# maropu/hivemall

Measured on AMD Instinct MI355X. Metric: rows/sec (node) FFM on Criteo-shaped sparse at 1/2/4/8 MI355X; logloss parity, higher is better.
Workload: dtype fp32

## Files before the change

### csrc/kernels/ffm.hip

```cpp
#include <type_traits>

#include "common.h"

namespace {

struct FFMParams {
    int B, F;
    int num_features, num_fields, Kp;
    int classification;
    int train;
    int use_linear, use_bias, norm;
    int reload;
    int gstride;
    int vpad;
    int tail16;
    int gfstride;
    int sstride;
    int fstride;
    long long vfe;
    uint32_t seed;
    float eta0, eps, lambda_v;
    float alpha, beta, lambda1, lambda2;
    float min_target, max_target;
    const void* reserved;
    int32_t* defer;
    int list_mode;
    int lin_defer;
    long long lstride;
    int lpack;
    int lin_atomic;
    const int32_t* hidx;
    const int32_t* hot_id;
    float* hacc;
    int nhot;
    int hacc_on;
    float* bias_sh;
    int bias_s;
    int bias_every;
};

#define LW(p, i) ((p)[(size_t)(i) * (size_t)P.lstride])

__device__ __forceinline__ float ftrl_weight(float z, float n, float alpha, float beta,
                                             float l1, float l2) {
    if (fabsf(z) <= l1) return 0.f;
    const float s = z > 0.f ? 1.f : -1.f;
    return -(z - s * l1) / ((beta + sqrtf(n)) / alpha + l2);
}

__device__ __forceinline__ float ftrl_update(float* __restrict__ z, float* __restrict__ n,
                                             float w, float g, float alpha, float beta,
                                             float l1, float l2) {
    const float n0 = *n;
    const float n1 = n0 + g * g;
    const float sigma = (sqrtf(n1) - sqrtf(n0)) / alpha;
    const float z1 = *z + g - sigma * w;
    *z = z1;
    *n = n1;
    return ftrl_weight(z1, n1, alpha, beta, l1, l2);
}

__device__ __forceinline__ float bias_w0(const FFMParams& P, const float* bias) {
    const float z = __hip_atomic_load(bias + 1, __ATOMIC_RELAXED, __HIP_MEMORY_SCOPE_AGENT);
    const float n = __hip_atomic_load(bias + 2, __ATOMIC_RELAXED, __HIP_MEMORY_SCOPE_AGENT);
    return ftrl_weight(z, n, P.alpha, P.beta, 0.f, 0.f);
}

__device__ __forceinline__ void bias_update(const FFMParams& P, float g, float* bias) {
    const float z0 = __hip_atomic_load(bias + 1, __ATOMIC_RELAXED, __HIP_MEMORY_SCOPE_AGENT);
    const float n0 = __hip_atomic_load(bias + 2, __ATOMIC_RELAXED, __HIP_MEMORY_SCOPE_AGENT);
    const float w = ftrl_weight(z0, n0, P.alpha, P.beta, 0.f, 0.f);
    const float sigma = (sqrtf(n0 + g * g) - sqrtf(n0)) / P.alpha;
    const float dz = g - sigma * w;
    atomicAdd(bias + 1, dz);
    atomicAdd(bias + 2, g * g);
    bias[0] = ftrl_weight(z0 + dz, n0 + g * g, P.alpha, P.beta, 0.f, 0.f);
}

__device__ __forceinline__ void bias_update_sh(const FFMParams& P, float g, float z0, float n0, float* sh,
                                               float* acc) {
    const float w = ftrl_weight(z0, n0, P.alpha, P.beta, 0.f, 0.f);
    const float sigma = (sqrtf(n0 + g * g) - sqrtf(n0)) / P.alpha;
    const float dz = g - sigma * w;
    atomicAdd(sh, dz);
    atomicAdd(sh + 1, g * g);
    acc[0] += dz;
    acc[1] += g * g;
}

constexpr int HD_SIZE = 2048;
constexpr int HD12_SIZE = 1024;
constexpr int HACC_STRIDE = 32;
constexpr int HACC_GRID = 2048;
constexpr int HACC_GRID12 = 2304;

__device__ __forceinline__ uint32_t hash3(uint32_t a, uint32_t b, uint32_t c) {
    uint32_t h = a * 0x9E3779B1u ^ (b + 0x7F4A7C15u) * 0x85EBCA77u ^ c * 0xC2B2AE3Du;
    h ^= h >> 15; h *= 0x2C1B3C6Du; h ^= h >> 12; h *= 0x297A2D39u; h ^= h >> 15;
    return h;
}

template <bool BF>
__device__ __forceinline__ float4 ld_chunk(const void* base, size_t off) {
    if constexpr (BF) {
        const uint2 q = *reinterpret_cast<const uint2*>(reinterpret_cast<const uint16_t*>(base) + off);
        return make_float4(__uint_as_float(q.x << 16), __uint_as_float(q.x & 0xFFFF0000u),
                           __uint_as_float(q.y << 16), __uint_as_float(q.y & 0xFFFF0000u));
    } else {
        return *reinterpret_cast<const float4*>(reinterpret_cast<const float*>(base) + off);
    }
}

template <bool BF>
__device__ __forceinline__ typename std::conditional<BF, uint2, float4>::type ld_raw(const void* base, size_t off) {
    if constexpr (BF) return *reinterpret_cast<const uint2*>(reinterpret_cast<const uint16_t*>(base) + off);
    else return *reinterpret_cast<const float4*>(reinterpret_cast<const float*>(base) + off);
}

template <bool BF, typename T>
__device__ __forceinline__ float4 to_f4(const T& q) {
    if constexpr (BF) {
        return make_float4(__uint_as_float(q.x << 16), __uint_as_float(q.x & 0xFFFF0000u),
                           __uint_as_float(q.y << 16), __uint_as_float(q.y & 0xFFFF0000u));
    } else {
        return q;
    }
}

template <bool BF>
__device__ __forceinline__ void st_chunk(void* base, size_t off, float4 v, uint32_t rnd) {
    if constexpr (BF) {
        const uint32_t r2 = rnd * 0x9E3779B1u + 0x632BE5ABu;
        const uint32_t lo = hm::pack_bf16x2_sr(v.x, rnd, v.y, rnd >> 16);
        const uint32_t hi = hm::pack_bf16x2_sr(v.z, r2, v.w, r2 >> 16);
        *reinterpret_cast<uint2*>(reinterpret_cast<uint16_t*>(base) + off) = make_uint2(lo, hi);
    } else {
        *reinterpret_cast<float4*>(reinterpret_cast<float*>(base) + off) = v;
    }
}

struct SlotMeta {
    int i, f;
    float x;
};

// ... 662 lines not shown
    if constexpr (PIN) asm("" : "+v"(m0), "+v"(m1), "+v"(m2), "+v"(m3));
    return m0 + m1 + m2 + m3;
}

constexpr int SG32_TRAIN = 1;

template <int NS, typename OT, int TPB = 256, int ATOM = 0, int KV = 1, int KEEP = 0, int LT = 0, int CFG = 0>
__global__ __launch_bounds__(TPB) __attribute__((amdgpu_waves_per_eu(TPB / 128))) void ffm_pipe_sg32_kernel(
    FFMParams P, const int32_t* __restrict__ idx, const int32_t* __restrict__ fld,
    const float* __restrict__ val, const float* __restrict__ y, void* __restrict__ Vt,
    float* __restrict__ Gt, float* __restrict__ w, float* __restrict__ wz, float* __restrict__ wn,
    float* __restrict__ bias, float* __restrict__ pred_out, float* __restrict__ loss_out)
{
    constexpr bool SPEC = (CFG & SG32_TRAIN) != 0;
    static_assert(!SPEC || (ATOM == 0 && KV == 1 && KEEP >= 2 && sizeof(OT) == 4 && TPB == 256),
                  "SG32_TRAIN: the default fp32 k <= 4 training launch only");
#define c_train (SPEC || P.train)
#define c_linear (SPEC || P.use_linear)
#define c_lpack (SPEC || P.lpack)
#define c_ldefer (SPEC || P.lin_defer)
#define c_bias (!SPEC && P.use_bias)
#define c_fld (SPEC || fld)
#define c_val (SPEC || val)
#define c_hacc (SPEC ? LT != 0 : P.hacc_on)
    __shared__ __attribute__((aligned(16))) float4 s_rv[NS * TPB * KV];
    __shared__ __attribute__((aligned(16))) float s_rg[NS * TPB];
    __shared__ __attribute__((aligned(16))) float4 s_t[NS * TPB * KV];
    __shared__ __attribute__((aligned(16))) int4 s_m[2][48];
    __shared__ __attribute__((aligned(16))) int s_mr[2][3][48];
    __shared__ __attribute__((aligned(16))) float s_lin[2][3][48];
    __shared__ __attribute__((aligned(16))) float4 s_lin4[2][48];
    __shared__ float s_red[TPB / 64 + 2];
    __shared__ int s_rep[TPB / 64];
    __shared__ float s_bias[4];
    __shared__ float s_bcur[2];
    __shared__ float2 s_hd[LT ? HD_SIZE : 1];
    __shared__ __attribute__((aligned(16))) float4 s_hacc[LT ? 2 : 1][48];
    __shared__ __attribute__((aligned(16))) int s_nh[LT ? 2 : 1][48];
    const int F = P.F;
    const int FF = F * F;
    const int tid = threadIdx.x, lane = tid & 63;
    const int wave = SPEC ? __builtin_amdgcn_readfirstlane(tid >> 6) : tid >> 6;
    constexpr int W_META = 1, W_LIN = 2, W_DMA = 3;
    const OT vfs = (OT)P.fstride * (16u * KV);
    const OT gfs = (OT)P.gstride * 4u;
    const int G = (int)gridDim.x;
    const int bid = (int)blockIdx.x;
    char* vb = reinterpret_cast<char*>(Vt);
    char* gb = reinterpret_cast<char*>(Gt);
    if constexpr (LT != 0) {
        for (int t = tid; t < HD_SIZE; t += TPB) s_hd[t] = make_float2(0.f, 0.f);
    }
    int nh = -1, kh = -1;

    int ab[NS];
    uint32_t okm = 0u;
#pragma unroll
    for (int j = 0; j < NS; ++j) {
        const int s = tid + j * TPB;
        if constexpr (SPEC) {
            const int a = s < FF ? s / F : 0, b = s < FF ? s % F : 0;
            ab[j] = (a << 4) | (b << 10) | ((s < FF ? b * F + a : s) << 16);
            okm |= (uint32_t)(s >= FF) << j | (uint32_t)(s >= FF || a == b) << (8 + j) | (uint32_t)(a < b) << (16 + j);
        } else {
            ab[j] = s < FF ? (s / F) | ((s % F) << 8) : 0;
        }
    }
#define SA(j) (SPEC ? (ab[j] >> 4) & 0x3F : ab[j] & 0xFF)
#define SB(j) (SPEC ? (ab[j] >> 10) & 0x3F : ab[j] >> 8)
#define ST(j) (SPEC ? ab[j] >> 16 : (SB(j) * F + SA(j)) * KV)

    auto dma_meta = [&](int bf, int row) {
        if (wave == W_DMA && lane < F && row < P.B) {
            const size_t o = (size_t)row * F + lane;
            __builtin_amdgcn_global_load_lds((glb_ptr_t)(idx + o), (lds_ptr_t)&s_mr[bf][0][0], 4, 0, 0);
            if (c_fld) __builtin_amdgcn_global_load_lds((glb_ptr_t)(fld + o), (lds_ptr_t)&s_mr[bf][1][0], 4, 0, 0);
            if (c_val) __builtin_amdgcn_global_load_lds((glb_ptr_t)(val + o), (lds_ptr_t)&s_mr[bf][2][0], 4, 0, 0);
        }
    };
    auto publish_meta = [&](int bf) {
        if (wave == W_META) {
            float sq = 0.f;
            if (lane < F) {
                int ri = s_mr[bf][0][lane];
                int rf = c_fld ? s_mr[bf][1][lane] : lane;
                float rx = c_val ? __int_as_float(s_mr[bf][2][lane]) : 1.f;
                if (ri < 0 || ri >= P.num_features || rf < 0 || rf >= P.num_fields) { ri = -1; rx = 0.f; rf = 0; }
                const int hb = SPEC && ri >= 0 ? (int)((uint32_t)ri * (uint32_t)vfs) : 0;
                s_m[bf][lane] = make_int4(ri, rf, __float_as_int(rx), hb);
                sq = rx * rx;
            }
            const float tot = hm::wave_sum_uniform(sq);
            if (lane == 0) s_red[TPB / 64 + bf] = (P.norm && tot > 0.f) ? rsqrtf(tot) : 1.f;
        }
    };
    auto slot = [&](int bf, int j, OT& ov, OT& og, float& xab) -> uint32_t {
        const int4 ma = s_m[bf][SA(j)], mb = s_m[bf][SB(j)];
        const bool ok = (ma.x | mb.x) >= 0 && tid + j * TPB < FF;
        const bool live = ok && SA(j) != SB(j);
        const OT i = ok ? (OT)(uint32_t)ma.x : (OT)0, f = ok ? (OT)(uint32_t)mb.y : (OT)0;
        ov = i * vfs + f * (16u * KV);
        og = i * gfs + f * 4u;
        xab = live ? __int_as_float(ma.z) * __int_as_float(mb.z) : 0.f;
        return live ? 1u : (ok ? 2u : 0u);
    };
    OT kov[KEEP ? NS : 1], kog[KEEP ? NS : 1], nov[KEEP ? NS : 1], nog[KEEP ? NS : 1];
// ... 9 lines not shown
                const int4 ma = s_m[bf][SA(j)], mb = s_m[bf][SB(j)];
                const int both = ma.x | mb.x;
                const bool ok = (both | (int)(okm << (31 - j))) >= 0;
                const bool live = (both | (int)(okm << (23 - j))) >= 0;
                const OT ib = ok ? (OT)(uint32_t)ma.w : (OT)0, f = ok ? (OT)(uint32_t)mb.y : (OT)0;
                OT f4 = f * 4u;
                asm("" : "+v"(f4));
                nov[j] = ib + f * 16u;
                nog[j] = ib + f4;
                nxab[j] = live ? __int_as_float(ma.z) * __int_as_float(mb.z) : 0.f;
                nwr |= (uint32_t)ok << j;
                eq |= (uint32_t)(ma.x == mb.x || ma.y == mb.y) << j;
                __builtin_amdgcn_global_load_lds((glb_ptr_t)(vb + nov[j]), (lds_ptr_t)(s_rv + j * TPB + wave * 64), 16, 0, 0);
                __builtin_amdgcn_global_load_lds((glb_ptr_t)(gb + nog[j]), (lds_ptr_t)(s_rg + j * TPB + wave * 64), 4, 0, 0);
            }
            nlive = nwr & ~(okm >> 8);
            if (P.defer) nrep = (int)(eq & nwr & (okm >> 16));
            return;
        }
#pragma unroll
        for (int j = 0; j < NS; ++j) {
            OT ov, og;
            float xab;
            const uint32_t k = slot(bf, j, ov, og, xab);
            if constexpr (KEEP) {
                nov[j] = ov;
                nog[j] = og;
                nxab[j] = xab;
                nlive |= (k & 1u) << j;
                nwr |= (uint32_t)(k != 0u) << j;
                if (P.defer) nrep |= (int)slot_repeats(SA(j), SB(j), s_m[bf][SA(j)], s_m[bf][SB(j)]);
            }
#pragma unroll
            for (int q = 0; q < KV; ++q)
                __builtin_amdgcn_global_load_lds((glb_ptr_t)(vb + ov + 16u * q),
                                                 (lds_ptr_t)(s_rv + (q * NS + j) * TPB + wave * 64), 16, 0, 0);
            __builtin_amdgcn_global_load_lds((glb_ptr_t)(gb + og), (lds_ptr_t)(s_rg + j * TPB + wave * 64), 4, 0, 0);
        }
    };
    auto keep_rotate = [&]() {
        if constexpr (KEEP) {
#pragma unroll
            for (int j = 0; j < NS; ++j) { kov[j] = nov[j]; kog[j] = nog[j]; kxab[j] = nxab[j]; }
            klive = nlive; kwr = nwr; krep = nrep;
        }
    };
    const int nlin = (c_linear && c_ldefer) ? ((c_lpack || !c_train) ? 1 + (LT != 0) : 3) : 0;
    auto dma_lin = [&](int bf) {
        if (c_linear && wave == W_LIN && lane < F) {
            const int i = max(s_m[bf][lane].x, 0);
            if (c_lpack) {
                __builtin_amdgcn_global_load_lds((glb_ptr_t)&LW(w, i), (lds_ptr_t)&s_lin4[bf][0], 16, 0, 0);
                if constexpr (LT != 0)
                    __builtin_amdgcn_global_load_lds((glb_ptr_t)(P.hacc + HACC_STRIDE * max(nh, 0)), (lds_ptr_t)&s_hacc[bf][0], 16, 0, 0);
                return;
            }
            __builtin_amdgcn_global_load_lds((glb_ptr_t)&LW(w, i), (lds_ptr_t)&s_lin[bf][0][0], 4, 0, 0);
            if (c_train) {
                __builtin_amdgcn_global_load_lds((glb_ptr_t)&LW(wz, i), (lds_ptr_t)&s_lin[bf][1][0], 4, 0, 0);
                __builtin_amdgcn_global_load_lds((glb_ptr_t)&LW(wn, i), (lds_ptr_t)&s_lin[bf][2][0], 4, 0, 0);
            }
        }
    };

    int row = bid;
    if (row >= P.B) return;
    if (tid == 0) { s_bcur[0] = 0.f; s_bcur[1] = 0.f; }
    dma_meta(0, row);
    __builtin_amdgcn_s_waitcnt(0x0F70);
    bar_raw();
    publish_meta(0);
    bar_raw();
    dma_slots(0);
    keep_rotate();
    if constexpr (LT != 0) {
        if (wave == W_LIN && lane < F) nh = s_m[0][lane].x >= 0 ? P.hidx[s_m[0][lane].x] : -1;
    }
    dma_lin(0);
    kh = nh;
    dma_meta(1, row + G);

    float4 fv[NS][KV];
    float fg[NS];
    OT fo[NS];
    uint32_t fwd = 0u;
    const bool bsh = c_bias && P.bias_sh;
    int bit = 0;
    float bz = 0.f, bn = 0.f;
    if (bsh && wave == W_META && lane < P.bias_s) {
        bz = __hip_atomic_load(P.bias_sh + lane * 32, __ATOMIC_RELAXED, __HIP_MEMORY_SCOPE_AGENT);
        bn = __hip_atomic_load(P.bias_sh + lane * 32 + 1, __ATOMIC_RELAXED, __HIP_MEMORY_SCOPE_AGENT);
    }
    for (int cur = 0; row < P.B; row += G, cur ^= 1) {
        const int nxt = cur ^ 1;
        const bool more = row + G < P.B;
        if constexpr (SPEC) asm volatile("" : "+v"(okm));
        if (wave == W_LIN && nlin == 3) __builtin_amdgcn_s_waitcnt(0x0F73);
        else if (wave == W_LIN && nlin == 2) __builtin_amdgcn_s_waitcnt(0x0F72);
        else if (wave == W_LIN && nlin == 1) __builtin_amdgcn_s_waitcnt(0x0F71);
        else __builtin_amdgcn_s_waitcnt(0x0F70);
        bar_raw();
        const bool bre = bsh && bit > 0 && (bit % P.bias_every) == 0;
        float nbz = bz, nbn = bn;
        if (bre && wave == W_META && lane < P.bias_s) {
            nbz = __hip_atomic_load(P.bias_sh + lane * 32, __ATOMIC_RELAXED, __HIP_MEMORY_SCOPE_AGENT);
            nbn = __hip_atomic_load(P.bias_sh + lane * 32 + 1, __ATOMIC_RELAXED, __HIP_MEMORY_SCOPE_AGENT);
        }
// ... 168 lines not shown
                            atomicAdd(vp + 4 * q + 2, e1.x);
                            atomicAdd(vp + 4 * q + 3, e1.y);
                        }
                        atomicAdd(reinterpret_cast<float*>(gb + og), gs - cg[j]);
                    }
                    continue;
                }
#pragma unroll
                for (int q = 0; q < KV; ++q) *reinterpret_cast<float4*>(vb + ov + 16u * q) = fv[j][q];
                *reinterpret_cast<float*>(gb + og) = fg[j];
            }
            if (mi >= 0) {
                if (c_linear) {
                    const float lz = hot ? hz : (c_lpack ? s_lin4[cur][lane].y : s_lin[cur][1][lane]);
                    const float ln = hot ? hn : (c_lpack ? s_lin4[cur][lane].z : s_lin[cur][2][lane]);
                    const float g = kappa * mx * scale;
                    const float n1 = ln + g * g;
                    const float z1 = lz + g - (sqrtf(n1) - sqrtf(ln)) / P.alpha * lw;
                    const float w1 = ftrl_weight(z1, n1, P.alpha, P.beta, P.lambda1, P.lambda2);
                    if (LT && hot) {
                        const float2 d = s_hd[kh];
                        s_hd[kh] = make_float2(d.x + (g - (sqrtf(n1) - sqrtf(ln)) / P.alpha * lw), d.y + g * g);
                    } else if (ATOM == 1) {
                        atomicAdd(&LW(wz, mi), z1 - lz);
                        atomicAdd(&LW(wn, mi), g * g);
                        LW(w, mi) = w1;
                    } else if (c_lpack) {
                        *reinterpret_cast<float4*>(&LW(w, mi)) = make_float4(w1, z1, n1, s_lin4[cur][lane].w);
                    } else {
                        LW(wz, mi) = z1;
                        LW(wn, mi) = n1;
                        LW(w, mi) = w1;
                    }
                }
            }
            if (c_bias && tid == 0) {
                if (bsh) bias_update_sh(P, kappa, s_bias[1], s_bias[2], P.bias_sh + (blockIdx.x % P.bias_s) * 32, s_bcur);
                else bias_update(P, kappa, bias);
            }
        }
        if constexpr (LT != 0) {
            if (more && wave == W_LIN && lane < F) nh = s_nh[nxt][lane];
        }
        if (more) dma_lin(nxt);
        kh = nh;
        keep_rotate();
        bz = nbz;
        bn = nbn;
        ++bit;
    }
    __builtin_amdgcn_s_waitcnt(0x0F70);
    if constexpr (LT != 0) {
        bar_raw();
        if (c_hacc)
            for (int t = tid; t < 2 * P.nhot; t += TPB) {
                const float2 d = s_hd[t >> 1];
                if (d.y != 0.f || d.x != 0.f) atomicAdd(P.hacc + HACC_STRIDE * (t >> 1) + (t & 1), (t & 1) ? d.y : d.x);
            }
    }
#undef SA
#undef SB
#undef ST
#undef c_train
#undef c_linear
#undef c_lpack
#undef c_ldefer
#undef c_bias
#undef c_fld
#undef c_val
#undef c_hacc
}

template <int NS, typename OT, int KEEP = 0, int LT = 0>
__global__ __launch_bounds__(256) __attribute__((amdgpu_waves_per_eu(4))) void ffm_pipe_sg12_kernel(
    FFMParams P, const int32_t* __restrict__ idx, const int32_t* __restrict__ fld,
    const float* __restrict__ val, const float* __restrict__ y, void* __restrict__ Vt,
    float* __restrict__ w, float* __restrict__ wz, float* __restrict__ wn,
    float* __restrict__ bias, float* __restrict__ pred_out, float* __restrict__ loss_out)
{
    __shared__ __attribute__((aligned(16))) uint32_t s_raw[NS * 256 * 4];
    __shared__ __attribute__((aligned(16))) uint2 s_t[NS * 256];
    __shared__ __attribute__((aligned(16))) int4 s_m[2][48];
    __shared__ __attribute__((aligned(16))) int s_mr[2][3][48];
    __shared__ __attribute__((aligned(16))) float s_lin[2][3][48];
    __shared__ __attribute__((aligned(16))) float4 s_lin4[2][48];
    __shared__ float s_red[8];
    __shared__ int s_rep[4];
    __shared__ float s_bias[4];
    __shared__ float s_bcur[2];
    __shared__ float2 s_hd[LT ? HD12_SIZE : 1];
    __shared__ __attribute__((aligned(16))) float4 s_hacc[LT ? 2 : 1][48];
    __shared__ __attribute__((aligned(16))) int s_nh[LT ? 2 : 1][48];
    const int F = P.F;
    const int FF = F * F;
    const int tid = threadIdx.x, wave = tid >> 6, lane = tid & 63;
    constexpr int W_META = 1, W_LIN = 2, W_DMA = 3;
    const OT bs = (OT)P.gstride * 4u;
    const int G = gridDim.x;
    char* vb = reinterpret_cast<char*>(Vt);
    if constexpr (LT != 0) {
        for (int t = tid; t < HD12_SIZE; t += 256) s_hd[t] = make_float2(0.f, 0.f);
    }
    int nh = -1, kh = -1;
    const bool lin_in_tail = reinterpret_cast<const char*>(w) == vb + (size_t)P.vpad * 12;
    typedef uint32_t u3v __attribute__((ext_vector_type(3)));

    int ab[NS];
#pragma unroll
    for (int j = 0; j < NS; ++j) {
        const int s = tid + j * 256;
        ab[j] = s < FF ? (s / F) | ((s % F) << 8) : 0;
    }
#define SA(j) (ab[j] & 0xFF)
#define SB(j) (ab[j] >> 8)
    const uint32_t tid_h = (uint32_t)tid * 0x9E3779B1u;

    auto dma_meta = [&](int bf, int row) {
        if (wave == W_DMA && lane < F && row < P.B) {
            const size_t o = (size_t)row * F + lane;
            __builtin_amdgcn_global_load_lds((glb_ptr_t)(idx + o), (lds_ptr_t)&s_mr[bf][0][0], 4, 0, 0);
            if (fld) __builtin_amdgcn_global_load_lds((glb_ptr_t)(fld + o), (lds_ptr_t)&s_mr[bf][1][0], 4, 0, 0);
            if (val) __builtin_amdgcn_global_load_lds((glb_ptr_t)(val + o), (lds_ptr_t)&s_mr[bf][2][0], 4, 0, 0);
        }
    };
    auto publish_meta = [&](int bf) {
        if (wave == W_META) {
            float sq = 0.f;
            if (lane < F) {
                int ri = s_mr[bf][0][lane];
                int rf = fld ? s_mr[bf][1][lane] : lane;
                float rx = val ? __int_as_float(s_mr[bf][2][lane]) : 1.f;
                if (ri < 0 || ri >= P.num_features || rf < 0 || rf >= P.num_fields) { ri = -1; rx = 0.f; rf = 0; }
                s_m[bf][lane] = make_int4(ri, rf, __float_as_int(rx), 0);
                sq = rx * rx;
            }
            const float tot = hm::wave_sum_uniform(sq);
            if (lane == 0) s_red[4 + bf] = (P.norm && tot > 0.f) ? rsqrtf(tot) : 1.f;
        }
    };
    auto slot = [&](int bf, int j, OT& off, float& xab) -> uint32_t {
        const int4 ma = s_m[bf][SA(j)], mb = s_m[bf][SB(j)];
        const bool ok = (ma.x | mb.x) >= 0 && tid + j * 256 < FF;
        const bool live = ok && SA(j) != SB(j);
        off = ok ? (OT)(uint32_t)ma.x * bs + (OT)(uint32_t)mb.y * 12u : (OT)0;
        xab = live ? __int_as_float(ma.z) * __int_as_float(mb.z) : 0.f;
        return live ? 1u : (ok ? 2u : 0u);
    };
    OT koff[KEEP ? NS : 1], noff[KEEP ? NS : 1];
    float kxab[KEEP ? NS : 1], nxab[KEEP ? NS : 1];
    uint32_t klive = 0u, kwr = 0u, nlive = 0u, nwr = 0u;
    int krep = 0, nrep = 0;
    auto dma_slots = [&](int bf) {
        if constexpr (KEEP) { nlive = 0u; nwr = 0u; nrep = 0; }
#pragma unroll
        for (int j = 0; j < NS; ++j) {
            OT off;
            float xab;
            const uint32_t k = slot(bf, j, off, xab);
            if constexpr (KEEP) {
                noff[j] = off;
                nxab[j] = xab;
                nlive |= (k & 1u) << j;
                nwr |= (uint32_t)(k != 0u) << j;
                if (P.defer) nrep |= (int)slot_repeats(SA(j), SB(j), s_m[bf][SA(j)], s_m[bf][SB(j)]);
            }
            __builtin_amdgcn_global_load_lds((glb_ptr_t)(vb + off), (lds_ptr_t)(s_raw + (j * 256 + wave * 64) * 4),
                                             12, 0, 0);
        }
    };
    auto keep_rotate = [&]() {
        if constexpr (KEEP) {
#pragma unroll
            for (int j = 0; j < NS; ++j) { koff[j] = noff[j]; kxab[j] = nxab[j]; }
            klive = nlive; kwr = nwr; krep = nrep;
        }
    };
    auto dma_lin = [&](int bf) {
        if (P.use_linear && wave == W_LIN && lane < F) {
            const int i = s_m[bf][lane].x;
            if (i >= 0 && P.lpack) {
                __builtin_amdgcn_global_load_lds((glb_ptr_t)&LW(w, i), (lds_ptr_t)&s_lin4[bf][0], 16, 0, 0);
                if (LT && nh >= 0)
                    __builtin_amdgcn_global_load_lds((glb_ptr_t)(P.hacc + HACC_STRIDE * nh), (lds_ptr_t)&s_hacc[bf][0], 16, 0, 0);
            } else if (i >= 0) {
                __builtin_amdgcn_global_load_lds((glb_ptr_t)&LW(w, i), (lds_ptr_t)&s_lin[bf][0][0], 4, 0, 0);
                if (P.train) {
                    __builtin_amdgcn_global_load_lds((glb_ptr_t)&LW(wz, i), (lds_ptr_t)&s_lin[bf][1][0], 4, 0, 0);
                    __builtin_amdgcn_global_load_lds((glb_ptr_t)&LW(wn, i), (lds_ptr_t)&s_lin[bf][2][0], 4, 0, 0);
                }
            }
        }
    };

    int row = blockIdx.x;
    if (row >= P.B) return;
    if (tid == 0) { s_bcur[0] = 0.f; s_bcur[1] = 0.f; }
    dma_meta(0, row);
    __builtin_amdgcn_s_waitcnt(0x0F70);
    bar_raw();
    publish_meta(0);
    bar_raw();
    dma_slots(0);
    keep_rotate();
    if constexpr (LT != 0) {
        if (P.hacc_on && wave == W_LIN && lane < F) nh = s_m[0][lane].x >= 0 ? P.hidx[s_m[0][lane].x] : -1;
    }
    dma_lin(0);
    kh = nh;
    dma_meta(1, row + G);

    const bool bsh = P.use_bias && P.bias_sh;
    int bit = 0;
    float bz = 0.f, bn = 0.f;
    if (bsh && wave == W_META && lane < P.bias_s) {
        bz = __hip_atomic_load(P.bias_sh + lane * 32, __ATOMIC_RELAXED, __HIP_MEMORY_SCOPE_AGENT);
        bn = __hip_atomic_load(P.bias_sh + lane * 32 + 1, __ATOMIC_RELAXED, __HIP_MEMORY_SCOPE_AGENT);
    }
    for (int cur = 0; row < P.B; row += G, cur ^= 1) {
        const int nxt = cur ^ 1;
        const bool more = row + G < P.B;
        __builtin_amdgcn_s_waitcnt(0x0F70);
        bar_raw();
        const bool bre = bsh && bit > 0 && (bit % P.bias_every) == 0;
        float nbz = bz, nbn = bn;
        if (bre && wave == W_META && lane < P.bias_s) {
            nbz = __hip_atomic_load(P.bias_sh + lane * 32, __ATOMIC_RELAXED, __HIP_MEMORY_SCOPE_AGENT);
            nbn = __hip_atomic_load(P.bias_sh + lane * 32 + 1, __ATOMIC_RELAXED, __HIP_MEMORY_SCOPE_AGENT);
        }
        if constexpr (LT != 0) {
            if (P.hacc_on && more && wave == W_LIN && lane < F) {
                const int ri = s_mr[nxt][0][lane];
                __builtin_amdgcn_global_load_lds((glb_ptr_t)(P.hidx + (ri >= 0 && ri < P.num_features ? ri : 0)),
                                                 (lds_ptr_t)&s_nh[nxt][0], 4, 0, 0);
            }
        }
        float cg[NS];
// ... 109 lines not shown
                o0 = o0 + rr * d0;
                o1 = o1 + rr * d1;
                const uint32_t h = rotl32(hrow, 5 * j + 1) ^ (0x9E3779B9u * (uint32_t)(j + 1));
                *reinterpret_cast<u3v*>(vb + off) = u3v{pack_sr_hi(o0, h, rotl32(h, 16)),
                                                        pack_sr_hi(o1, rotl32(h, 8), rotl32(h, 24)),
                                                        __float_as_uint(gs)};
            }
            {
                const int npad = P.vpad - P.num_fields;
                const int per = npad + P.tail16;
                for (int q = tid; q < F * per; q += 256) {
                    const int a = q / per, kk = q - a * per;
                    const int i = s_m[cur][a].x;
                    if (i < 0) continue;
                    char* blk = vb + (OT)(uint32_t)i * bs;
                    if (kk < npad) *reinterpret_cast<u3v*>(blk + (P.num_fields + kk) * 12) = u3v{0u, 0u, 0u};
                    else if (!(lin_in_tail && kk == npad))
                        *reinterpret_cast<uint4*>(blk + P.vpad * 12 + 16 * (kk - npad)) = make_uint4(0u, 0u, 0u, 0u);
                }
            }
            if (mi >= 0 && P.use_linear) {
                const float lz = hot ? hz : (P.lpack ? s_lin4[cur][lane].y : s_lin[cur][1][lane]);
                const float ln = hot ? hn : (P.lpack ? s_lin4[cur][lane].z : s_lin[cur][2][lane]);
                const float g = kappa * mx * scale;
                const float n1 = ln + g * g;
                const float z1 = lz + g - (sqrtf(n1) - sqrtf(ln)) / P.alpha * lw;
                const float w1 = ftrl_weight(z1, n1, P.alpha, P.beta, P.lambda1, P.lambda2);
                if (LT && hot) {
                    const float2 d = s_hd[kh];
                    s_hd[kh] = make_float2(d.x + (g - (sqrtf(n1) - sqrtf(ln)) / P.alpha * lw), d.y + g * g);
                } else if (P.lpack) {
                    *reinterpret_cast<float4*>(&LW(w, mi)) = make_float4(w1, z1, n1, 0.f);
                } else {
                    LW(wz, mi) = z1;
                    LW(wn, mi) = n1;
                    LW(w, mi) = w1;
                }
            }
            if (P.use_bias && tid == 0) {
                if (bsh) bias_update_sh(P, kappa, s_bias[1], s_bias[2], P.bias_sh + (blockIdx.x % P.bias_s) * 32, s_bcur);
                else bias_update(P, kappa, bias);
            }
        }
        if (more) dma_lin(nxt);
        kh = nh;
        keep_rotate();
        bz = nbz;
        bn = nbn;
        ++bit;
    }
    __builtin_amdgcn_s_waitcnt(0x0F70);
    if constexpr (LT != 0) {
        bar_raw();
        if (P.hacc_on)
            for (int t = tid; t < 2 * P.nhot; t += 256) {
                const float2 d = s_hd[t >> 1];
                if (d.y != 0.f || d.x != 0.f) atomicAdd(P.hacc + HACC_STRIDE * (t >> 1) + (t & 1), (t & 1) ? d.y : d.x);
            }
    }
#undef SA
#undef SB
}


int default_blocks(int B, int grid, int cap = 256 * 8 * 4) {
    return grid > 0 ? grid : (B < cap ? B : cap);
}

struct FFMArgs {
    const int32_t *idx, *fld;
    const float *val, *y;
    void *V, *G;
    float *w, *wz, *wn, *bias, *pred, *loss;
};

using KernelV = void (*)(FFMParams, const int32_t*, const int32_t*, const float*, const float*, void*,
                         float*, float*, float*, float*, float*, float*);
template <typename GT>
using KernelVG = void (*)(FFMParams, const int32_t*, const int32_t*, const float*, const float*, void*, GT*,
                          float*, float*, float*, float*, float*, float*);

void launch(KernelV k, int blocks, int tpb, size_t lds, hipStream_t stream, const FFMParams& P, const FFMArgs& a) {
    hipLaunchKernelGGL(k, dim3(blocks), dim3(tpb), lds, stream, P, a.idx, a.fld, a.val, a.y, a.V, a.w, a.wz, a.wn,
                       a.bias, a.pred, a.loss);
}
template <typename GT>
void launch(KernelVG<GT> k, int blocks, int tpb, size_t lds, hipStream_t stream, const FFMParams& P, const FFMArgs& a) {
    hipLaunchKernelGGL(k, dim3(blocks), dim3(tpb), lds, stream, P, a.idx, a.fld, a.val, a.y, a.V,
                       reinterpret_cast<GT*>(a.G), a.w, a.wz, a.wn, a.bias, a.pred, a.loss);
}

template <int N0, int... NR, typename Fn>
void with_ns(int need, Fn&& f) {
    if constexpr (sizeof...(NR) == 0) f(std::integral_constant<int, N0>{});
    else if (need <= N0) f(std::integral_constant<int, N0>{});
    else with_ns<NR...>(need, f);
}

template <bool BF>
int dispatch_lean(const FFMParams& P, const FFMArgs& a, int grid, hipStream_t stream) {
    const size_t slot_b = BF ? 16 : 32;
    if (P.Kp != 4 || P.F > 45) return -1;
    if ((size_t)P.num_features * (size_t)P.fstride * slot_b >= ((size_t)1 << 32)) return -1;
    const size_t lean_lds = (size_t)P.F * P.F * 16 + (size_t)P.F * 16 + 16 * 4;
    const int need = (P.F * P.F + 255) / 256;
    const int blocks = default_blocks(P.B, grid);
    if (blocks <= 0) return 0;
    with_ns<2, 4, 6, 8>(need, [&](auto ns) {
        constexpr int NS = decltype(ns)::value;
        if constexpr (BF) launch(ffm_pipe_kernel<NS>, blocks, 256, 0, stream, P, a);
        else launch(ffm_lean_kernel<NS>, blocks, 256, lean_lds, stream, P, a);
    });
    HM_LAUNCH_RET();
}

__global__ __launch_bounds__(256) void ffm_hacc_kernel(FFMParams P, float* __restrict__ w, int dir) {
    const int h = blockIdx.x * 256 + threadIdx.x;
    if (h >= P.nhot) return;
    float4* rp = reinterpret_cast<float4*>(&LW(w, P.hot_id[h]));
    float4* ap = reinterpret_cast<float4*>(P.hacc + HACC_STRIDE * h);
    const float4 r = *rp;
    if (dir == 0) {
        *ap = make_float4(r.y, r.z, 0.f, 0.f);
    } else {
        const float4 a = *ap;
        const float nw = a.y > 0.f ? ftrl_weight(a.x, a.y, P.alpha, P.beta, P.lambda1, P.lambda2) : r.x;
        *rp = make_float4(nw, a.x, a.y, r.w);
    }
}

template <typename Fn>
int with_side_table(const FFMParams& Q, float* w, hipStream_t stream, Fn&& train) {
    if (Q.hacc_on) {
        hipLaunchKernelGGL(ffm_hacc_kernel, dim3((Q.nhot + 255) / 256), dim3(256), 0, stream, Q, w, 0);
        HM_LAUNCH_RET_IF_ERR();
    }
    train();
    if (Q.hacc_on) {
        HM_LAUNCH_RET_IF_ERR();
        hipLaunchKernelGGL(ffm_hacc_kernel, dim3((Q.nhot + 255) / 256), dim3(256), 0, stream, Q, w, 1);
    }
    HM_LAUNCH_RET();
}

int dispatch_sg12(const FFMParams& P, const FFMArgs& a, int grid, hipStream_t stream) {
    if (P.Kp != 4 || P.F > 45) return -1;
    const bool wide = (size_t)P.num_features * (size_t)P.gstride * 4 >= ((size_t)1 << 32);
    const int need = (P.F * P.F + 255) / 256;
    int blocks = default_blocks(P.B, grid, 256 * 8 * 8);
    if (blocks <= 0) return 0;
    FFMParams Q = P;
    Q.hacc_on = P.lin_atomic == 4 && P.lin_defer && P.nhot <= HD12_SIZE && blocks > 1 && !wide;
    if (Q.hacc_on && grid <= 0) blocks = default_blocks(P.B, grid, HACC_GRID12);
    return with_side_table(Q, a.w, stream, [&] {
        with_ns<2, 4, 6, 8>(need, [&](auto ns) {
            constexpr int NS = decltype(ns)::value;
            if (wide) launch(ffm_pipe_sg12_kernel<NS, uint64_t>, blocks, 256, 0, stream, Q, a);
            else if (Q.hacc_on) launch(ffm_pipe_sg12_kernel<NS, uint32_t, 2, 1>, blocks, 256, 0, stream, Q, a);
            else launch(ffm_pipe_sg12_kernel<NS, uint32_t, 2>, blocks, 256, 0, stream, Q, a);
        });
    });
}

int dispatch_sg32(const FFMParams& P, const FFMArgs& a, int grid, int variant, hipStream_t stream) {
    if ((P.Kp != 4 && P.Kp != 8) || P.F > 45 || P.vpad <= 0) return -1;
    const bool wide = (size_t)P.num_features * (size_t)P.fstride * (size_t)(P.Kp * 4) >= ((size_t)1 << 32) ||
                      (size_t)P.num_features * (size_t)P.gstride * 4 >= ((size_t)1 << 32);
    const int tpb = P.Kp == 8 ? 512 : 256;
    const int need = (P.F * P.F + tpb - 1) / tpb;
    int blocks = default_blocks(P.B, grid);
    if (blocks <= 0) return 0;
    FFMParams Q = P;
    Q.hacc_on = P.lin_atomic == 4 && P.lin_defer && blocks > 1 && !wide && variant != 6;
    if (Q.hacc_on && grid <= 0) blocks = default_blocks(P.B, grid, HACC_GRID);
    if (P.Kp == 8)
        return with_side_table(Q, a.w, stream, [&] {
            with_ns<2, 3, 4>(need, [&](auto ns) {
                constexpr int NS = decltype(ns)::value;
// ... 36 lines not shown
        case 2: return launch_ffm<2, BF, SG>(P, a, grid, stream);
        case 3: return launch_ffm<3, BF, SG>(P, a, grid, stream);
        case 4: return launch_ffm<4, BF, SG>(P, a, grid, stream);
        case 8: return launch_ffm<8, BF, SG>(P, a, grid, stream);
        default: return (int)hipErrorInvalidValue;
    }
}

template <bool BF>
int dispatch(const FFMParams& P, const FFMArgs& a, int grid, int packed, int slot_g, int variant,
             hipStream_t stream, int* fast) {
    *fast = 1;
    if (slot_g) {
        if (P.gfstride == 3) {
            if (!BF) return (int)hipErrorInvalidValue;
            const int rc = variant == 1 ? -1 : dispatch_sg12(P, a, grid, stream);
            if (rc != -1) return rc;
            *fast = 0;
            return launch_generic<true, true>(P, a, grid, stream);
        }
        if (variant != 1 && !BF && P.gfstride == 1) {
            const int rc = dispatch_sg32(P, a, grid, variant, stream);
            if (rc != -1) return rc;
        }
        *fast = 0;
        return launch_generic<BF, true>(P, a, grid, stream);
    }
    if (packed && variant != 1) {
        const int rc = dispatch_lean<BF>(P, a, grid, stream);
        if (rc != -1) return rc;
    }
    *fast = 0;
    return launch_generic<BF, false>(P, a, grid, stream);
}

constexpr int DEFER_BLOCKS = 512;

template <bool BF>
int launch_deferred(FFMParams P, const FFMArgs& a, int slot_g, int grid_req, hipStream_t stream) {
    P.list_mode = 1;
    const int cap = grid_req > 0 && grid_req < DEFER_BLOCKS ? grid_req : DEFER_BLOCKS;
    const int grid = P.B < cap ? P.B : cap;
    return slot_g ? launch_generic<BF, true>(P, a, grid, stream) : launch_generic<BF, false>(P, a, grid, stream);
}

}

HM_API int hm_ffm_step(const int32_t* ip, const float* hp, const int32_t* idx, const int32_t* fld,
                       const float* val, const float* y, void* V, void* G, float* w, float* wz,
                       float* wn, float* bias, float* pred, float* loss, void* const* aux,
                       hipStream_t stream) {
    const FFMArgs a{idx, fld, val, y, V, G, w, wz, wn, bias, pred, loss};
    FFMParams P;
    P.reserved = nullptr;
    P.defer = aux ? reinterpret_cast<int32_t*>(aux[1]) : nullptr;
    P.list_mode = 0;
    P.B = ip[0]; P.F = ip[1]; P.num_features = ip[2]; P.num_fields = ip[3]; P.Kp = ip[4];
    P.classification = ip[5]; P.train = ip[6]; P.use_linear = ip[7]; P.use_bias = ip[8];
    P.norm = ip[9];
    const int grid = ip[10];
    P.reload = ip[11];
    const int bf16 = ip[12];
    P.seed = (uint32_t)ip[13];
    const int packed = ip[14];
    const int variant = ip[15];
    if (variant != 0 && variant != 1 && variant != 6 && variant != 11) return (int)hipErrorInvalidValue;
    if (ip[26] != 0 && ip[26] != 4) return (int)hipErrorInvalidValue;
    P.sstride = packed ? 2 * P.Kp : P.Kp;
    P.fstride = ip[16] > 0 ? ip[16] : P.num_fields;
    const int slot_g = ip[17];
    P.gstride = ip[18];
    P.vpad = ip[19];
    P.tail16 = ip[20];
    P.gfstride = ip[21] > 0 ? ip[21] : 1;
    P.lin_defer = ip[22];
    P.lstride = ip[24] > 0 ? ip[24] : 1;
    P.lpack = ip[25];
    P.lin_atomic = P.lpack ? ip[26] : 0;
    P.hidx = nullptr; P.hot_id = nullptr; P.hacc = nullptr; P.nhot = 0; P.hacc_on = 0;

    if (P.lin_atomic == 4) {
        P.nhot = ip[27];
        if (aux) {
            P.hidx = reinterpret_cast<const int32_t*>(aux[4]);
            P.hot_id = reinterpret_cast<const int32_t*>(aux[5]);
            P.hacc = reinterpret_cast<float*>(aux[6]);
        }
        if (!P.hidx || !P.hot_id || !P.hacc || P.nhot <= 0 || P.nhot > HD_SIZE || !P.train || !P.use_linear)
            P.lin_atomic = 0;
    }
    if (P.lpack && (wz != w + 1 || wn != w + 2 || (P.lstride & 3) || (reinterpret_cast<uintptr_t>(w) & 15)))
        return (int)hipErrorInvalidValue;
    P.bias_sh = aux ? reinterpret_cast<float*>(aux[2]) : nullptr;
    P.bias_s = aux ? (int)reinterpret_cast<intptr_t>(aux[3]) : 0;
    if (!P.bias_sh || P.bias_s < 1 || P.bias_s > 64 || !P.train) { P.bias_sh = nullptr; P.bias_s = 0; }
    P.bias_every = ip[23] > 0 ? ip[23] : 16;
    if (P.fstride < P.num_fields) return (int)hipErrorInvalidValue;
    P.vfe = (long long)P.fstride * P.sstride;
    P.eta0 = hp[0]; P.eps = hp[1]; P.lambda_v = hp[2]; P.alpha = hp[3]; P.beta = hp[4];
    P.lambda1 = hp[5]; P.lambda2 = hp[6]; P.min_target = hp[7]; P.max_target = hp[8];
    if (P.F <= 0 || P.F > 256 || (P.Kp & 3)) return (int)hipErrorInvalidValue;
    if (slot_g) {
        if (packed || P.gstride < P.num_fields || P.tail16 < 0) return (int)hipErrorInvalidValue;
        if (P.gfstride == 3) {
            if (!bf16 || P.Kp != 4 || reinterpret_cast<char*>(G) != reinterpret_cast<char*>(V) + 8 ||
                P.vpad < P.num_fields || (size_t)P.vpad * 12 + (size_t)P.tail16 * 16 != (size_t)P.gstride * 4)
                return (int)hipErrorInvalidValue;
            P.sstride = 6;
            P.vfe = (long long)P.gstride * 2;
        } else if (P.vpad > 0) {
            const size_t es = bf16 ? 2 : 4;
            if (reinterpret_cast<char*>(G) != reinterpret_cast<char*>(V) + (size_t)P.vpad * P.Kp * es ||
                (size_t)P.fstride * P.Kp * es != (size_t)P.gstride * 4 || P.vpad < P.num_fields ||
                P.gfstride != 1)
                return (int)hipErrorInvalidValue;
        }
    } else if (packed) {
        const size_t es = bf16 ? 2 : 4;
        if (reinterpret_cast<char*>(G) != reinterpret_cast<char*>(V) + (size_t)P.Kp * es)
            return (int)hipErrorInvalidValue;
        if ((size_t)P.num_features * (size_t)P.fstride >= ((size_t)1 << 32)) return (int)hipErrorInvalidValue;
    }
    if (!P.train || P.B <= 0) P.defer = nullptr;
    if (P.defer) {
        const hipError_t e = hipMemsetAsync(P.defer, 0, sizeof(int32_t), stream);
        if (e != hipSuccess) return (int)e;
    }
    int fast = 0;
    const int rc = bf16 ? dispatch<true>(P, a, grid, packed, slot_g, variant, stream, &fast)
                        : dispatch<false>(P, a, grid, packed, slot_g, variant, stream, &fast);
    if (rc != 0 || !fast || !P.defer) return rc;
    return bf16 ? launch_deferred<true>(P, a, slot_g, grid, stream) : launch_deferred<false>(P, a, slot_g, grid, stream);
}
```

### hivemall_amd/ops/ffm.py

```python
from __future__ import annotations

import ctypes
import os
from dataclasses import dataclass

import numpy as np
import torch

from .. import _native


@dataclass
class FFMHyper:
    eta0: float = 0.2
    eps: float = 1.0
    lambda_v: float = 1e-4
    alpha: float = 0.2
    beta: float = 1.0
    lambda1: float = 1e-3
    lambda2: float = 1e-4
    min_target: float = -3.4e38
    max_target: float = 3.4e38
    classification: bool = True
    use_linear: bool = True
# ... 91 lines not shown


def new_state_tables(num_features: int, num_fields: int, kp: int, dtype, device,
                     packed: bool, slot_g: bool = False) -> tuple[torch.Tensor, torch.Tensor]:
    if slot_g:
        if packed and dtype == torch.bfloat16 and kp == 4:
            fs, bs = slot12_layout(num_fields)
            buf = torch.zeros((num_features, bs), dtype=torch.uint8, device=device)
            sl = buf[:, :fs * 12]
            V = sl.view(torch.bfloat16).view(num_features, fs, 6)[:, :num_fields, :4]
            G = sl.view(torch.float32).view(num_features, fs, 3)[:, :num_fields, 2]
            return V, G
        if packed:
            fs, bs, goff = slot_block_layout(num_fields, kp, dtype)
            es = torch.empty(0, dtype=dtype).element_size()
            buf = torch.zeros((num_features, bs), dtype=torch.uint8, device=device)
            V = buf[:, :goff].view(dtype).view(num_features, fs, kp)[:, :num_fields]
            G = buf[:, goff:goff + fs * 4].view(torch.float32)[:, :num_fields]
            assert V.stride(0) * es == bs and G.stride(0) * 4 == bs
            return V, G
        return (torch.zeros((num_features, num_fields, kp), dtype=dtype, device=device),
                torch.zeros((num_features, num_fields), dtype=torch.float32, device=device))
    if packed:
        fs = padded_fields(num_fields, kp, dtype)
        VG = torch.zeros((num_features, fs, 2, kp), dtype=dtype, device=device)
        return VG[:, :num_fields, 0, :], VG[:, :num_fields, 1, :]
    shape = (num_features, num_fields, kp)
    return (torch.zeros(shape, dtype=dtype, device=device),
            torch.zeros(shape, dtype=dtype, device=device))


_DEFER: dict = {}
BIAS_SHARDS = int(os.environ.get("HM_FFM_BIAS_SHARDS", "64"))
BIAS_EVERY = int(os.environ.get("HM_FFM_BIAS_EVERY", "32"))
_BIAS_SH: dict = {}


def _launch_key(device: torch.device):
    return (device, _native.stream_of(device))


def _bias_shards(device: torch.device) -> torch.Tensor:
    key = _launch_key(device)
    sh = _BIAS_SH.get(key)
    if sh is None or sh.shape[0] != BIAS_SHARDS:
        sh = torch.zeros((BIAS_SHARDS, 32), dtype=torch.float32, device=device)
        _BIAS_SH[key] = sh
    return sh
_DEFER_ON = os.environ.get("HM_FFM_DEFER", "1") != "0"
_LIN_DEFER = int(os.environ.get("HM_FFM_LIN_DEFER", "1") != "0")
LIN_MODES = (0, 4)
_LIN_ATOMIC = int(os.environ.get("HM_FFM_LIN_ATOMIC", "4"))
_LIN_HOT_N = min(int(os.environ.get("HM_FFM_LIN_HOT", "2048")), 2048)
_LIN_HOT: dict = {}
_LIN_HOT_KEEP = 8


_LIN_HOT_REFRESH = int(os.environ.get("HM_FFM_LIN_HOT_REFRESH", "256"))


def _lin_hot_tables(state: dict, idx: torch.Tensor, nhot: int):
    w = state["w"]
    nf = w.shape[0]
    key = (w.device, w.data_ptr(), nf, nhot)
    t = _LIN_HOT.get(key)
    if t is not None:
        t[3][0] += 1
        if _LIN_HOT_REFRESH > 0 and t[3][0] % _LIN_HOT_REFRESH == 0:
            del _LIN_HOT[key]
            t = None
    if t is None:
        cnt = torch.bincount(idx.reshape(-1).long().clamp(0, nf - 1), minlength=nf)
        top = torch.argsort(cnt, descending=True)[:nhot]
        top = top[cnt[top] > 0].to(torch.int32)
        hidx = torch.full((nf,), -1, dtype=torch.int32, device=w.device)
        hidx[top.long()] = torch.arange(top.numel(), dtype=torch.int32, device=w.device)
        hacc = torch.zeros(max(1, top.numel()), 32, dtype=torch.float32, device=w.device)
        while len(_LIN_HOT) >= _LIN_HOT_KEEP:
            _LIN_HOT.pop(next(iter(_LIN_HOT)))
        t = _LIN_HOT[key] = (hidx, top, hacc, [0])
    return t[:3]


def _defer_buffer(device: torch.device, B: int) -> torch.Tensor:
    key = _launch_key(device)
    buf = _DEFER.get(key)
    if buf is None or buf.numel() < 1 + B:
        buf = torch.empty(1 + max(B, 1 << 16), dtype=torch.int32, device=device)
        _DEFER[key] = buf
    return buf


def _has_multihot(idx: torch.Tensor, fld: torch.Tensor | None) -> bool:
    if idx.numel() == 0 or idx.shape[1] < 2:
        return False
    big = torch.iinfo(torch.int32).max
    pos = torch.arange(idx.shape[1], device=idx.device, dtype=torch.int32)

    def rep(t: torch.Tensor, valid: torch.Tensor) -> bool:
        u = torch.where(valid, t, big - pos.unsqueeze(0))
        s = u.sort(dim=1).values
        return bool((s[:, 1:] == s[:, :-1]).any().item())

    valid = idx >= 0
    if rep(idx, valid):
        return True
    return fld is not None and rep(fld, valid & (fld >= 0))


def ffm_step(state: dict, idx: torch.Tensor, fld: torch.Tensor | None, val: torch.Tensor | None,
             y: torch.Tensor | None, hyper: FFMHyper, train: bool = True,
             pred: torch.Tensor | None = None, loss: torch.Tensor | None = None,
             grid: int = 0, variant: int | None = None, lin_mode: int | None = None) -> None:
    auto = variant is None and _VARIANT == 0
    variant = _VARIANT if variant is None else int(variant)
    lin_mode = _LIN_ATOMIC if lin_mode is None else int(lin_mode)
    for what, v, live in (("kernel variant", variant, VARIANTS), ("linear mode", lin_mode, LIN_MODES)):
        if v not in live:
            raise ValueError(f"FFM {what} {v}: the live values are {live}")
    V = state["V"]
    B, F = idx.shape
    NF, NFLD, Kp = V.shape
    assert idx.dtype == torch.int32 and idx.is_contiguous()
    for t in (fld, val, y, pred, loss):
        if t is not None:
            assert t.device == V.device and t.is_contiguous(), "tensor device/layout mismatch"
    if fld is not None:
        assert fld.dtype == torch.int32 and fld.shape == idx.shape
    if val is not None:
        assert val.dtype == torch.float32 and val.shape == idx.shape
    if y is not None:
        assert y.shape[0] == B
    if pred is not None:
        assert pred.shape[0] >= B
# ... 2 lines not shown
    if V.is_cuda and train and int(grid) == 1 and auto and _has_multihot(idx, fld):
        variant = 1
    G = state["G"]
    bf16 = V.dtype == torch.bfloat16
    slot_g = G.dim() == 2
    gstride = 0
    block = (0, 0)
    if slot_g:
        assert G.dtype == torch.float32 and G.shape == V.shape[:2] and G.stride(1) in (1, 3), \
            "per-slot G: fp32 [num_features, num_fields], field stride 1 (or 3: 12-B bf16 slots)"
        assert V.stride(2) == 1 and (V.stride(1) == Kp or (G.stride(1) == 3 and V.stride(1) == 6)), \
            "V: [NF, FS, Kp] slots (or the V part of 12-B {V | G} slots)"
        packed = False
        gstride = G.stride(0)
        es = V.element_size()
        d = G.data_ptr() - V.data_ptr()
        bs = V.stride(0) * es
        if G.stride(1) == 3:
            fs, bs12 = slot12_layout(NFLD)
            assert V.is_cuda and bf16 and d == 8 and G.stride(0) * 4 == bs12, "12-B slot layout"
            block = (fs, (bs12 - fs * 12) // 16)
        elif V.is_cuda and G.stride(1) == 1 and 0 < d < bs and d % (Kp * es) == 0 and G.stride(0) * 4 == bs:
            vpad = d // (Kp * es)
            tail = bs - d - vpad * 4
            if tail >= 0 and tail % 16 == 0:
                block = (vpad, tail // 16)
    else:
        assert G.dtype == V.dtype, "V and G must share the storage dtype"
        packed = is_packed(V, G)
        if not packed:
            assert V.is_contiguous() and G.is_contiguous(), \
                "FFM state: two contiguous V/G tables or the halves of one packed table"
    assert not bf16 or V.is_cuda, "bf16 FFM state is a device-only layout"
    global _CALLS
    _CALLS += 1
    ip = np.array([B, F, NF, NFLD, Kp, int(hyper.classification), int(train), int(hyper.use_linear),
                   int(hyper.use_bias), int(hyper.norm), int(grid),
                   int((not packed) if hyper.reload is None else hyper.reload), int(bf16),
                   (hyper.seed * 1000003 + _CALLS) & 0x7FFFFFFF, int(packed), variant,
                   field_stride(V), int(slot_g), gstride, block[0], block[1],
                   G.stride(1) if slot_g else 0, _LIN_DEFER, BIAS_EVERY] + list(_lin_addressing(state))
                  + [lin_mode, 0], dtype=np.int32)
    hp = hyper.hp()
    p = _native.ptr
    args = (ip.ctypes.data, hp.ctypes.data, p(idx), p(fld), p(val), p(y), p(V), p(G),
            p(state["w"]), p(state["wz"]), p(state["wn"]), p(state["bias"]), p(pred), p(loss))
    if V.is_cuda:
        bsh = _bias_shards(V.device) if (train and hyper.use_bias and BIAS_SHARDS > 0) else None
        if bsh is not None:
            b = state["bias"]
            zn0 = b[1:3].clone()
            bsh.zero_()
            bsh[0, :2] = zn0
        hidx = hot_id = hacc = None
        if lin_mode == 4 and train and hyper.use_linear and _lin_addressing(state)[1]:
            hidx, hot_id, hacc = _lin_hot_tables(state, idx, 1024 if bf16 else _LIN_HOT_N)
        nhot = hot_id.numel() if hot_id is not None else 0
        ip[26], ip[27] = lin_mode if nhot else 0, nhot
        aux = (ctypes.c_void_p * 7)(None, p(_defer_buffer(V.device, B)) if (train and _DEFER_ON) else None,
                                    p(bsh), bsh.shape[0] if bsh is not None else 0,
                                    p(hidx), p(hot_id), p(hacc))
        rc = _native.hip().hm_ffm_step(*args, ctypes.addressof(aux), _native.stream_of(V.device))
        _native.check(rc, "hm_ffm_step")
        if bsh is not None:
            b[1:3] = bsh[:, :2].sum(0) + (b[1:3] - zn0)
        if train and hyper.use_bias:
            b = state["bias"]
            b[0] = -b[1] / ((hyper.beta + b[2].sqrt()) / hyper.alpha)
    else:
        rc = _native.host().hm_ffm_step_cpu(*args)
        if rc != 0:
            raise RuntimeError(f"hm_ffm_step_cpu failed: {rc}")
```

Baseline: 94.76 million.

## Compact hot-feature accumulator and add per-XCD read replicas for linear updates

The hot linear-weight accumulator shrinks from a 32-float stride to 2 floats per entry. Hot-weight reads in the pipeline now come from 8 per-XCD replica tables (hread), which are refreshed at block end from the accumulator using atomic loads. The flush step uses a wave ballot so that atomics are only issued for 64-byte segments with nonzero deltas. This targets atomic contention and cross-XCD cache traffic on hot rows, in exchange for more false sharing on the compact table, extra replica writes at every block end, and reads of state that may be stale.

New measurement: 92.38 million. -2.5%, worse.

```diff
diff --git a/csrc/kernels/ffm.hip b/csrc/kernels/ffm.hip
--- a/csrc/kernels/ffm.hip
+++ b/csrc/kernels/ffm.hip
@@ -22,7 +22,7 @@
     float eta0, eps, lambda_v;
     float alpha, beta, lambda1, lambda2;
     float min_target, max_target;
-    const void* reserved;
+    float* hread;
     int32_t* defer;
     int list_mode;
     int lin_defer;
@@ -90,7 +90,42 @@
 
 constexpr int HD_SIZE = 2048;
 constexpr int HD12_SIZE = 1024;
-constexpr int HACC_STRIDE = 32;
+constexpr int HACC_STRIDE = 2;
+static_assert(HACC_STRIDE == 2 || HACC_STRIDE == 4 || HACC_STRIDE == 8, "8-B aligned entries, whole 64-B segments");
+constexpr int HREAD_COPIES = 8;
+constexpr int HREAD_EVERY = 1;
+
+__device__ __forceinline__ int xcd_id() {
+    return (int)(__builtin_amdgcn_s_getreg((3 << 11) | 20) & (HREAD_COPIES - 1));
+}
+
+template <int TPB>
+__device__ __forceinline__ void side_table_flush(const FFMParams& P, const float2* s_hd, float4* hrd, int bid) {
+    const int tid = threadIdx.x, lane = tid & 63;
+    constexpr int SEG = 32 / HACC_STRIDE;
+    const int n2 = 2 * P.nhot;
+    for (int t0 = 0; t0 < n2; t0 += TPB) {
+        const int t = t0 + tid;
+        const float2 d = t < n2 ? s_hd[t >> 1] : make_float2(0.f, 0.f);
+        const unsigned long long nz = __ballot(d.x != 0.f || d.y != 0.f);
+        if (t < n2 && ((nz >> (lane & ~(SEG - 1))) & ((1ull << SEG) - 1ull)) != 0ull)
+            atomicAdd(P.hacc + HACC_STRIDE * (t >> 1) + (t & 1), (t & 1) ? d.y : d.x);
+    }
+    if (HREAD_EVERY > 1 && (bid / HREAD_COPIES) % HREAD_EVERY != 0) return;
+    constexpr int U = 8;
+    for (int h0 = tid; h0 < P.nhot; h0 += U * TPB) {
+        unsigned long long zn[U];
+#pragma unroll
+        for (int u = 0; u < U; ++u)
+            if (h0 + u * TPB < P.nhot)
+                zn[u] = __hip_atomic_load(reinterpret_cast<const unsigned long long*>(P.hacc + HACC_STRIDE * (h0 + u * TPB)),
+                                          __ATOMIC_RELAXED, __HIP_MEMORY_SCOPE_AGENT);
+#pragma unroll
+        for (int u = 0; u < U; ++u)
+            if (h0 + u * TPB < P.nhot)
+                hrd[h0 + u * TPB] = make_float4(__uint_as_float((uint32_t)zn[u]), __uint_as_float((uint32_t)(zn[u] >> 32)), 0.f, 0.f);
+    }
+}
 constexpr int HACC_GRID = 2048;
 constexpr int HACC_GRID12 = 2304;
 
@@ -859,6 +894,7 @@
         for (int t = tid; t < HD_SIZE; t += TPB) s_hd[t] = make_float2(0.f, 0.f);
     }
     int nh = -1, kh = -1;
+    float4* hrd = LT != 0 ? reinterpret_cast<float4*>(P.hread) + (size_t)xcd_id() * (size_t)P.nhot : nullptr;
 
     int ab[NS];
     uint32_t okm = 0u;
@@ -974,7 +1010,7 @@
             if (c_lpack) {
                 __builtin_amdgcn_global_load_lds((glb_ptr_t)&LW(w, i), (lds_ptr_t)&s_lin4[bf][0], 16, 0, 0);
                 if constexpr (LT != 0)
-                    __builtin_amdgcn_global_load_lds((glb_ptr_t)(P.hacc + HACC_STRIDE * max(nh, 0)), (lds_ptr_t)&s_hacc[bf][0], 16, 0, 0);
+                    __builtin_amdgcn_global_load_lds((glb_ptr_t)(hrd + max(nh, 0)), (lds_ptr_t)&s_hacc[bf][0], 16, 0, 0);
                 return;
             }
             __builtin_amdgcn_global_load_lds((glb_ptr_t)&LW(w, i), (lds_ptr_t)&s_lin[bf][0][0], 4, 0, 0);
@@ -1249,11 +1285,7 @@
     __builtin_amdgcn_s_waitcnt(0x0F70);
     if constexpr (LT != 0) {
         bar_raw();
-        if (c_hacc)
-            for (int t = tid; t < 2 * P.nhot; t += TPB) {
-                const float2 d = s_hd[t >> 1];
-                if (d.y != 0.f || d.x != 0.f) atomicAdd(P.hacc + HACC_STRIDE * (t >> 1) + (t & 1), (t & 1) ? d.y : d.x);
-            }
+        if (c_hacc) side_table_flush<TPB>(P, s_hd, hrd, bid);
     }
 #undef SA
 #undef SB
@@ -1299,6 +1331,7 @@
         for (int t = tid; t < HD12_SIZE; t += 256) s_hd[t] = make_float2(0.f, 0.f);
     }
     int nh = -1, kh = -1;
+    float4* hrd = LT != 0 ? reinterpret_cast<float4*>(P.hread) + (size_t)xcd_id() * (size_t)P.nhot : nullptr;
     const bool lin_in_tail = reinterpret_cast<const char*>(w) == vb + (size_t)P.vpad * 12;
     typedef uint32_t u3v __attribute__((ext_vector_type(3)));
 
@@ -1378,7 +1411,7 @@
             if (i >= 0 && P.lpack) {
                 __builtin_amdgcn_global_load_lds((glb_ptr_t)&LW(w, i), (lds_ptr_t)&s_lin4[bf][0], 16, 0, 0);
                 if (LT && nh >= 0)
-                    __builtin_amdgcn_global_load_lds((glb_ptr_t)(P.hacc + HACC_STRIDE * nh), (lds_ptr_t)&s_hacc[bf][0], 16, 0, 0);
+                    __builtin_amdgcn_global_load_lds((glb_ptr_t)(hrd + nh), (lds_ptr_t)&s_hacc[bf][0], 16, 0, 0);
             } else if (i >= 0) {
                 __builtin_amdgcn_global_load_lds((glb_ptr_t)&LW(w, i), (lds_ptr_t)&s_lin[bf][0][0], 4, 0, 0);
                 if (P.train) {
@@ -1594,11 +1627,7 @@
     __builtin_amdgcn_s_waitcnt(0x0F70);
     if constexpr (LT != 0) {
         bar_raw();
-        if (P.hacc_on)
-            for (int t = tid; t < 2 * P.nhot; t += 256) {
-                const float2 d = s_hd[t >> 1];
-                if (d.y != 0.f || d.x != 0.f) atomicAdd(P.hacc + HACC_STRIDE * (t >> 1) + (t & 1), (t & 1) ? d.y : d.x);
-            }
+        if (P.hacc_on) side_table_flush<256>(P, s_hd, hrd, (int)blockIdx.x);
     }
 #undef SA
 #undef SB
@@ -1660,12 +1689,14 @@
     const int h = blockIdx.x * 256 + threadIdx.x;
     if (h >= P.nhot) return;
     float4* rp = reinterpret_cast<float4*>(&LW(w, P.hot_id[h]));
-    float4* ap = reinterpret_cast<float4*>(P.hacc + HACC_STRIDE * h);
+    float2* ap = reinterpret_cast<float2*>(P.hacc + HACC_STRIDE * h);
     const float4 r = *rp;
     if (dir == 0) {
-        *ap = make_float4(r.y, r.z, 0.f, 0.f);
+        *ap = make_float2(r.y, r.z);
+        for (int c = 0; c < HREAD_COPIES; ++c)
+            reinterpret_cast<float4*>(P.hread)[(size_t)c * P.nhot + h] = make_float4(r.y, r.z, 0.f, 0.f);
     } else {
-        const float4 a = *ap;
+        const float2 a = *ap;
         const float nw = a.y > 0.f ? ftrl_weight(a.x, a.y, P.alpha, P.beta, P.lambda1, P.lambda2) : r.x;
         *rp = make_float4(nw, a.x, a.y, r.w);
     }
@@ -1808,7 +1839,7 @@
                        hipStream_t stream) {
     const FFMArgs a{idx, fld, val, y, V, G, w, wz, wn, bias, pred, loss};
     FFMParams P;
-    P.reserved = nullptr;
+    P.hread = nullptr;
     P.defer = aux ? reinterpret_cast<int32_t*>(aux[1]) : nullptr;
     P.list_mode = 0;
     P.B = ip[0]; P.F = ip[1]; P.num_features = ip[2]; P.num_fields = ip[3]; P.Kp = ip[4];
@@ -1838,11 +1869,12 @@
     if (P.lin_atomic == 4) {
         P.nhot = ip[27];
         if (aux) {
+            P.hread = reinterpret_cast<float*>(aux[0]);
             P.hidx = reinterpret_cast<const int32_t*>(aux[4]);
             P.hot_id = reinterpret_cast<const int32_t*>(aux[5]);
             P.hacc = reinterpret_cast<float*>(aux[6]);
         }
-        if (!P.hidx || !P.hot_id || !P.hacc || P.nhot <= 0 || P.nhot > HD_SIZE || !P.train || !P.use_linear)
+        if (!P.hidx || !P.hot_id || !P.hacc || !P.hread || P.nhot <= 0 || P.nhot > HD_SIZE || !P.train || !P.use_linear)
             P.lin_atomic = 0;
     }
     if (P.lpack && (wz != w + 1 || wn != w + 2 || (P.lstride & 3) || (reinterpret_cast<uintptr_t>(w) & 15)))
diff --git a/hivemall_amd/ops/ffm.py b/hivemall_amd/ops/ffm.py
--- a/hivemall_amd/ops/ffm.py
+++ b/hivemall_amd/ops/ffm.py
@@ -167,6 +167,8 @@
 LIN_MODES = (0, 4)
 _LIN_ATOMIC = int(os.environ.get("HM_FFM_LIN_ATOMIC", "4"))
 _LIN_HOT_N = min(int(os.environ.get("HM_FFM_LIN_HOT", "2048")), 2048)
+_HACC_STRIDE = 2
+_HREAD_COPIES = 8
 _LIN_HOT: dict = {}
 _LIN_HOT_KEEP = 8
 
@@ -190,11 +192,12 @@
         top = top[cnt[top] > 0].to(torch.int32)
         hidx = torch.full((nf,), -1, dtype=torch.int32, device=w.device)
         hidx[top.long()] = torch.arange(top.numel(), dtype=torch.int32, device=w.device)
-        hacc = torch.zeros(max(1, top.numel()), 32, dtype=torch.float32, device=w.device)
+        hacc = torch.zeros(max(1, top.numel()), _HACC_STRIDE, dtype=torch.float32, device=w.device)
+        hread = torch.zeros(_HREAD_COPIES, max(1, top.numel()), 4, dtype=torch.float32, device=w.device)
         while len(_LIN_HOT) >= _LIN_HOT_KEEP:
             _LIN_HOT.pop(next(iter(_LIN_HOT)))
-        t = _LIN_HOT[key] = (hidx, top, hacc, [0])
-    return t[:3]
+        t = _LIN_HOT[key] = (hidx, top, hacc, [0], hread)
+    return t[0], t[1], t[2], t[4]
 
 
 def _defer_buffer(device: torch.device, B: int) -> torch.Tensor:
@@ -303,12 +306,12 @@
             zn0 = b[1:3].clone()
             bsh.zero_()
             bsh[0, :2] = zn0
-        hidx = hot_id = hacc = None
+        hidx = hot_id = hacc = hread = None
         if lin_mode == 4 and train and hyper.use_linear and _lin_addressing(state)[1]:
-            hidx, hot_id, hacc = _lin_hot_tables(state, idx, 1024 if bf16 else _LIN_HOT_N)
+            hidx, hot_id, hacc, hread = _lin_hot_tables(state, idx, min(1024, _LIN_HOT_N) if bf16 else _LIN_HOT_N)
         nhot = hot_id.numel() if hot_id is not None else 0
         ip[26], ip[27] = lin_mode if nhot else 0, nhot
-        aux = (ctypes.c_void_p * 7)(None, p(_defer_buffer(V.device, B)) if (train and _DEFER_ON) else None,
+        aux = (ctypes.c_void_p * 7)(p(hread), p(_defer_buffer(V.device, B)) if (train and _DEFER_ON) else None,
                                     p(bsh), bsh.shape[0] if bsh is not None else 0,
                                     p(hidx), p(hot_id), p(hacc))
         rc = _native.hip().hm_ffm_step(*args, ctypes.addressof(aux), _native.stream_of(V.device))
```
